# Syclus123/xDeepFM-pytorch

Measured on AMD Instinct MI355X. Metric: examples/sec (xDeepFM train step, Criteo-shape synthetic, bs=4096 per GPU), higher is better.
Workload: dtype f32

## Files before the change

xdeepfm-pytorch_amd/csrc/api.hip:

```cpp
#include <stdlib.h>
#include <string.h>
#include <algorithm>
#include <vector>
#include "xdfm_internal.h"
#include "finish_batch.h"

static thread_local char g_err[512] = "";
static int g_opts[OPT_COUNT] = {
     1,
     0,
     1,
     0,
     0,
     1,
     0,
     0,
     0,
     0,
     0,
     -1,
     -1,
     -1,
     0,
     1,
     1,
     -1,
     -1,
     -1,
     -1,
     -1,
     -1,
     1,
     -1,
     0,
     1,
     7,
     -1,
     -1,
     -1,
};
static const char* const g_opt_names[OPT_COUNT] = {"fwd_nf", "bww_nsplit", "bww_slab", "bww_mt", "dbg", "cin_math", "x3_fwd_mt", "x3_bwx_rows", "x3_waves", "bww_phase", "adam_bx", "last_fwd_kernel", "last_bwx_kernel", "last_bww_kernel", "last_sym", "x3_sym", "bww_xcd", "last_fwd_inst", "last_bwx_inst", "last_bww_inst", "last_fwd_f32", "last_bwx_f32", "last_bww_f32", "adam_rows", "last_adam_rows", "opt_bx", "finish_batch", "colaunch", "last_colaunch", "last_riders", "last_pack_riders"};

int xdfm_fail(int code, const char* fmt, ...) {
    va_list ap;
    va_start(ap, fmt);
    vsnprintf(g_err, sizeof(g_err), fmt, ap);
    va_end(ap);
    return code;
}

int xdfm_opt(int idx) { return g_opts[idx]; }

#define XDFM_MAX_DEVICES 16
void xdfm_opt_note(int idx, int value) { g_opts[idx] = value; }

__global__ __launch_bounds__(FINISH_THREADS) void finish_multi_kernel(const FinishTable tab) {
    __shared__ float smf[FINISH_THREADS];
    __shared__ double smd[4];
    int ji = 0;
#pragma unroll
    for (int k = 1; k < FINISH_MAX_JOBS; ++k) ji += (int)blockIdx.x >= tab.first[k] ? 1 : 0;
    const FinishJob& j = tab.j[ji];
    const int lb = (int)blockIdx.x - tab.first[ji];
    bool scalar_out = false;
    switch (j.kind) {
        case FJ_CIN_DBIAS:
            cin_dbias_finish_row(lb * FINISH_THREADS + (int)threadIdx.x, (const float*)j.part, j.i0, j.i1, (float*)j.out, j.i2 != 0);
            break;
        case FJ_DENSE_W:
            if (lb < j.i1) dn_finish_elem((long)lb * FINISH_THREADS + threadIdx.x, (const float*)j.part, j.i0, j.n0, j.n1, (float*)j.out, (float*)j.out2);
            else dn_dalpha_finish_block((const double*)j.part2, j.i2, (float*)j.out3, smd);
            break;
        case FJ_COLSUM:
            colsum_finish_block(lb, (const float*)j.part, j.i0, (float*)j.out, smf);
            break;
        case FJ_HEAD_FWD:
            head_fwd_finish_block((const float*)j.part, smf);
            if (threadIdx.x == 0) ((float*)j.out)[0] = smf[0];
            scalar_out = true;
            break;
        case FJ_HEAD_BWD:
            head_bwd_finish_elem(lb * FINISH_THREADS + (int)threadIdx.x, (const float*)j.part, j.i0, (float*)j.out);
            break;
        case FJ_ADAM_L2:
            adam_l2_finish_block<FINISH_THREADS>((const float*)j.part, j.i0, smf);
            if (threadIdx.x == 0) {
                ((float*)j.out)[0] = smf[0];
                if (j.cell) adam_rows_finish_one(j.cell, (float*)j.out);
            }
            scalar_out = true;
            break;
        case FJ_ADAM_ROWS:
            if (threadIdx.x == 0) adam_rows_finish_one(j.cell, (float*)j.out);
            scalar_out = true;
            break;
        default:
            scalar_out = true;
            break;
    }
    if (scalar_out && threadIdx.x == 0 && j.add_out) j.add_out[0] = j.add_a[0] + j.add_b[0];
}

struct FinishBatch {
    std::vector<FinishJob> jobs;
    hipStream_t st = nullptr;
};
static FinishBatch g_finish[XDFM_MAX_DEVICES];
static int g_finish_dev = -1;

static bool finish_job_writes(const FinishJob& j, const void* p) {
    return p && (j.out == p || j.out2 == p || j.out3 == p || (const void*)j.add_out == p || (const void*)j.cell == p);
}

static int finish_launch_pending(FinishBatch& fb) {
    const size_t n = fb.jobs.size();
    for (size_t j0 = 0; j0 < n; j0 += FINISH_MAX_JOBS) {
        FinishTable tab;
        memset(&tab, 0, sizeof(tab));
        tab.n = (int)(n - j0 < FINISH_MAX_JOBS ? n - j0 : FINISH_MAX_JOBS);
        std::stable_sort(fb.jobs.begin() + j0, fb.jobs.begin() + j0 + tab.n,
                         [](const FinishJob& a, const FinishJob& b) { return a.blocks < b.blocks; });
        int blocks = 0;
        for (int k = 0; k < tab.n; ++k) {
            tab.j[k] = fb.jobs[j0 + k];
            tab.first[k] = blocks;
            blocks += tab.j[k].blocks;
        }
        for (int k = tab.n; k <= FINISH_MAX_JOBS; ++k) tab.first[k] = blocks;
        if (blocks > 0) hipLaunchKernelGGL(finish_multi_kernel, dim3(blocks), dim3(FINISH_THREADS), 0, fb.st, tab);
    }
    fb.jobs.clear();
    return xdfm_check_launch("finish_batch");
}

int xdfm_finish_defer(const FinishJob& job, hipStream_t st, bool* taken) {
    *taken = false;
    if (g_finish_dev < 0) return XDFM_OK;
    int dev = -1;
    if (hipGetDevice(&dev) != hipSuccess || dev != g_finish_dev)
        return xdfm_fail(XDFM_ERR_INVALID, "finish batch: opened on device %d, a finish arrives on device %d", g_finish_dev, dev);
    FinishBatch& fb = g_finish[dev];
    if (fb.jobs.empty()) fb.st = st;
    else if (fb.st != st)
        return xdfm_fail(XDFM_ERR_INVALID, "finish batch: a finish arrives on stream %p, the batch collects on stream %p", (void*)st, (void*)fb.st);
    XDFM_REQUIRE(job.blocks > 0 && job.kind >= 0 && job.kind < FJ_KINDS, "finish batch: bad job (kind %d, %d workgroups)", job.kind, job.blocks);
    *taken = true;
    if (job.kind == FJ_ADAM_ROWS && job.out)
        for (size_t k = fb.jobs.size(); k-- > 0;)
            if (fb.jobs[k].kind == FJ_ADAM_L2 && fb.jobs[k].out == job.out && !fb.jobs[k].cell && !fb.jobs[k].add_out) {
                fb.jobs[k].cell = job.cell;
                return XDFM_OK;
            }
    if (job.kind == FJ_ADD)
        for (size_t k = fb.jobs.size(); k-- > 0;) {
            FinishJob& p = fb.jobs[k];
            if ((p.kind == FJ_ADAM_L2 || p.kind == FJ_ADAM_ROWS) && p.out && p.out == (const void*)job.add_b && !p.add_out &&
                !finish_job_writes(p, job.add_a)) {
                p.add_a = job.add_a; p.add_b = job.add_b; p.add_out = job.add_out;
                return XDFM_OK;
            }
        }
    const void* reads[4] = {nullptr, nullptr, nullptr, nullptr};
    if (job.kind == FJ_ADAM_ROWS) { reads[0] = job.out; reads[1] = job.cell; }
    if (job.kind == FJ_ADD) { reads[0] = job.add_a; reads[1] = job.add_b; }
    if (job.kind == FJ_CIN_DBIAS && !job.i2) reads[0] = job.out;
    reads[2] = job.out; reads[3] = job.add_out;
    bool clash = false;
    for (const FinishJob& p : fb.jobs)
        for (const void* r : reads) clash = clash || finish_job_writes(p, r);
    if (clash)
        if (int rc = finish_launch_pending(fb)) return rc;
    fb.jobs.push_back(job);
    return XDFM_OK;
}

__global__ void finish_add_kernel(const float* a, const float* b, float* out) {
    if (threadIdx.x == 0 && blockIdx.x == 0) out[0] = a[0] + b[0];
}

extern "C" {

int xdfm_abi_version(void) { return XDFM_ABI_VERSION; }

const char* xdfm_last_error(void) { return g_err; }

int xdfm_device_count(void) {
    int n = 0;
    hipError_t e = hipGetDeviceCount(&n);
    return e == hipSuccess ? n : -(int)e;
}

int xdfm_graph_node_census(void* graph, int* n_nodes, int* n_memset, int* n_unexpected) {
    if (!graph || !n_nodes || !n_memset || !n_unexpected) return xdfm_fail(XDFM_ERR_INVALID, "graph_node_census: null pointer");
    size_t n = 0;
// ... 119 lines not shown
```

xdeepfm-pytorch_amd/csrc/embed.hip:

```cpp
#include "xdfm_internal.h"
#include "cin_x3_pack.h"
#include "rider.h"

#define EMB_THREADS 256

template <int VEC>
__global__ __launch_bounds__(EMB_THREADS) void embed_gather_kernel(
    const float* __restrict__ X, long ldx, int B, const float* const* __restrict__ tables,
    const float* const* __restrict__ lin_tables, const int* __restrict__ cols, const int* __restrict__ vocab,
    int m, int D, const int* __restrict__ dense_cols, const float* __restrict__ dense_w, int nd, int EB,
    float* __restrict__ emb_fm, float* __restrict__ dnn_in, long ldd, int dense_off, float* __restrict__ lin_out,
    int* __restrict__ err_flag, int own_blocks, const X3PackJobs riders) {
    if ((int)blockIdx.x >= own_blocks) { x3_pack_rider(riders, (long)((int)blockIdx.x - own_blocks)); return; }
    extern __shared__ __attribute__((aligned(16))) float smem[];
    float* tile = smem;
    float* linv = smem + (size_t)EB * m * D;
    const float** rowp = reinterpret_cast<const float**>(smem + ((((size_t)EB * m * (D + 1)) + 1) & ~(size_t)1));
    float* densev = reinterpret_cast<float*>(rowp + (size_t)EB * m);
    float* wl = densev + (size_t)EB * nd;
    const int tid = threadIdx.x;
    const int b0 = blockIdx.x * EB;
    const int nb = (B - b0 < EB) ? B - b0 : EB;
    const int DV = D / VEC;
    const long N = (long)B * D;

    const int ndense = nb * nd;
    float dval[2] = {0.f, 0.f};
    float wval = 0.f;
    if (nd > 0) {
#pragma unroll
        for (int t = 0; t < 2; ++t) {
            const int idx = tid + t * EMB_THREADS;
            const int c = idx < ndense ? idx : 0;
            const int bl = c / nd, k = c - bl * nd;
            dval[t] = X[(long)(b0 + bl) * ldx + dense_cols[k]];
        }
        if (dense_w) wval = dense_w[tid < nd ? tid : 0];
    }
    const int npass = m <= 32 ? (nb + 7) / 8 : (nb * m + EMB_THREADS - 1) / EMB_THREADS;
    for (int p = 0; p < npass; ++p) {
        int jf, bl;
        if (m <= 32) { jf = tid & 31; bl = (tid >> 5) + 8 * p; }
        else { const int rj = tid + p * EMB_THREADS; bl = rj / m; jf = rj - bl * m; }
        const bool live = jf < m && bl < nb;
        const int jc = live ? jf : 0, bc = live ? bl : 0;
        const float* tab = tables[jc];
        const float* ltab = lin_tables ? lin_tables[jc] : tab;
        const int V = vocab[jc];
        long id = (long)X[(long)(b0 + bc) * ldx + cols[jc]];
        if (id < 0 || id >= V) {
            if (err_flag && live) atomicOr(err_flag, 1);
            id = id < 0 ? 0 : V - 1;
        }
        const float lv = ltab[lin_tables ? id : 0];
        if (live) {
            rowp[bl * m + jf] = tab + id * D;
            if (lin_tables) linv[bl * m + jf] = lv;
        }
    }
    if (nd > 0) {
#pragma unroll
        for (int t = 0; t < 2; ++t)
            if (tid + t * EMB_THREADS < ndense) densev[tid + t * EMB_THREADS] = dval[t];
        for (int idx = tid + 2 * EMB_THREADS; idx < ndense; idx += EMB_THREADS) {
            const int bl = idx / nd, k = idx - bl * nd;
            densev[idx] = X[(long)(b0 + bl) * ldx + dense_cols[k]];
        }
        if (dense_w) {
            if (tid < nd) wl[tid] = wval;
            for (int k = tid + EMB_THREADS; k < nd; k += EMB_THREADS) wl[k] = dense_w[k];
        }
    }
    __syncthreads();
    const int nchunks = nb * m * DV;
    const bool dv_pow2 = (DV & (DV - 1)) == 0;
    const int dv_sh = 31 - __builtin_clz(DV);
    constexpr int GB = 8;
    for (int base = 0; base < nchunks; base += GB * EMB_THREADS) {
        float4 v[GB];
        int at[GB];
#pragma unroll
        for (int k = 0; k < GB; ++k) {
            const int idx = base + k * EMB_THREADS + tid;
            const int cidx = idx < nchunks ? idx : nchunks - 1;
            const int rj = dv_pow2 ? (cidx >> dv_sh) : (cidx / DV);
            const int q = cidx - rj * DV;
            const float* src = rowp[rj] + q * VEC;
            at[k] = idx < nchunks ? rj * D + q * VEC : -1;
            if constexpr (VEC == 4) {
                v[k] = *reinterpret_cast<const float4*>(src);
            } else if constexpr (VEC == 2) {
                const float2 t = *reinterpret_cast<const float2*>(src);
                v[k] = make_float4(t.x, t.y, 0.f, 0.f);
            } else {
                v[k] = make_float4(*src, 0.f, 0.f, 0.f);
            }
        }
#pragma unroll
        for (int k = 0; k < GB; ++k) {
            if (at[k] < 0) continue;
            float* dst = tile + at[k];
            if constexpr (VEC == 4) *reinterpret_cast<float4*>(dst) = v[k];
            else if constexpr (VEC == 2) *reinterpret_cast<float2*>(dst) = make_float2(v[k].x, v[k].y);
            else *dst = v[k].x;
        }
    }
    __syncthreads();

    if (dnn_in) {
        const int per = m * D;
        for (int bl = 0; bl < nb; ++bl) {
            float* drow = dnn_in + (long)(b0 + bl) * ldd;
            const float* trow = tile + (size_t)bl * per;
            for (int k = tid; k < per; k += EMB_THREADS) drow[k] = trow[k];
            for (int k = tid; k < nd; k += EMB_THREADS) drow[dense_off + k] = densev[bl * nd + k];
        }
    }
    {
        const int per = nb * D;
        const bool d_pow2 = (D & (D - 1)) == 0;
        const int d_sh = 31 - __builtin_clz(D);
        for (int k = tid; k < per; k += EMB_THREADS) {
            const int bl = d_pow2 ? (k >> d_sh) : (k / D);
            const float* src = tile + (size_t)bl * m * D + (k - bl * D);
            float* dst = emb_fm + (long)b0 * D + k;
            for (int j = 0; j < m; ++j) dst[(long)j * N] = src[j * D];
        }
    }
    if (lin_out && tid < nb) {
        float acc = 0.f;
        if (lin_tables)
            for (int j = 0; j < m; ++j) acc += linv[tid * m + j];
        float dacc = 0.f;
        for (int k = 0; k < nd; ++k) dacc += densev[tid * nd + k] * wl[k];
        lin_out[b0 + tid] = acc + dacc;
    }
}

#define SC_THREADS 512
#define SC_ROWS 4096
#define SC_W 8
#define SC_SW 4
#define SC_RIDER_BLOCKS 512
#define SC_NC 4
#define SC_EMPTY 0xffffffffu

typedef float f4u __attribute__((ext_vector_type(4), aligned(4)));

__device__ __forceinline__ int sc_scale_exp(float amax) {
    const int E = (int)((__float_as_uint(amax) >> 23) & 0xff);
    return 37 - ((E == 0 ? 1 : E) - 127);
}
__device__ __forceinline__ double sc_pow2(int s) { return __longlong_as_double((long long)(1023 + s) << 52); }
__device__ __forceinline__ double sc_fix(float v, double sc) { return __builtin_rint((double)v * sc); }

__host__ __device__ inline size_t sc_lds_bytes(int npad) {
    const size_t hash = (size_t)2 * npad * 2 * sizeof(unsigned);
    const size_t slots = (size_t)(npad / SC_W) * 2 * (SC_NC * (sizeof(double) + sizeof(float)) + 2 * sizeof(int));
    return (hash > slots ? hash : slots) + (size_t)(npad + 8) * (sizeof(unsigned) + sizeof(unsigned short)) + 64 +
           (size_t)npad * 4 * sizeof(float);
}

static_assert(sizeof(X3UnpackRiders) + 512 <= 8192, "embed_scatter_grouped_kernel's argument block");
template <int VEC>
__global__ __launch_bounds__(SC_THREADS) void embed_scatter_grouped_kernel(
    const float* __restrict__ X, long ldx, int b0, int nb, long Btot, const int* __restrict__ cols,
    const int* __restrict__ vocab, int m, int D, int nslice, const float* __restrict__ d_emb_fm,
    const float* __restrict__ d_dnn_in, long ld_dnn, const float* __restrict__ d_lin, long ld_lin,
    float* __restrict__ d_flat, const long* __restrict__ tab_off, const long* __restrict__ lin_off,
    unsigned char* __restrict__ marks, int npad, int nlin, const int* __restrict__ dense_cols, int nd,
    float* __restrict__ d_dense_w, long dense_mark_base, int dbg, int own_blocks, const X3UnpackRiders riders) {
    if ((int)blockIdx.x >= own_blocks) { x3_unpack_rider(riders, (long)((int)blockIdx.x - own_blocks)); return; }
    extern __shared__ __attribute__((aligned(16))) char sc_smem[];
    const int tid = threadIdx.x;

    if ((int)blockIdx.x >= m * nslice + nlin) {
        const int k = blockIdx.x - m * nslice - nlin;
        const int col = dense_cols[k];
        float* red = reinterpret_cast<float*>(sc_smem);
        double* redd = reinterpret_cast<double*>(sc_smem + 64);
        constexpr int PER = SC_ROWS / SC_THREADS;
        float p[PER];
        float mx = 0.f;
#pragma unroll
        for (int t = 0; t < PER; ++t) {
            const int bl = tid + t * SC_THREADS;
            const long b = b0 + (bl < nb ? bl : 0);
            const float x = X[b * ldx + col], g = d_lin[b * ld_lin];
            p[t] = bl < nb ? x * g : 0.f;
            mx = fmaxf(mx, fabsf(p[t]));
        }
        for (int o = 32; o > 0; o >>= 1) mx = fmaxf(mx, __shfl_xor(mx, o));
        if ((tid & 63) == 0) red[tid >> 6] = mx;
        __syncthreads();
        mx = 0.f;
#pragma unroll
        for (int t = 0; t < SC_THREADS / 64; ++t) mx = fmaxf(mx, red[t]);
        const int s = sc_scale_exp(mx);
        const double sc = sc_pow2(s);
        double acc = 0.0;
#pragma unroll
        for (int t = 0; t < PER; ++t) acc += sc_fix(p[t], sc);
        for (int o = 32; o > 0; o >>= 1) acc += __shfl_xor(acc, o);
        if ((tid & 63) == 0) redd[tid >> 6] = acc;
        __syncthreads();
        if (tid == 0) {
            acc = 0.0;
#pragma unroll
            for (int t = 0; t < SC_THREADS / 64; ++t) acc += redd[t];
            d_dense_w[k] += (float)(acc * sc_pow2(-s));
            if (marks) marks[(dense_mark_base + k) >> 2] = 1;
        }
        return;
    }

    const bool lin = (int)blockIdx.x >= m * nslice;
    const int j = lin ? (int)blockIdx.x - m * nslice : (int)blockIdx.x / nslice;
    const int slice = lin ? 0 : (int)blockIdx.x - j * nslice;
    const int nwin = npad / SC_W;
    const int HS = 2 * npad;
    unsigned* tkey = reinterpret_cast<unsigned*>(sc_smem);
    unsigned* tcnt = tkey + HS;
    double* seqS = reinterpret_cast<double*>(sc_smem);
    float* seqM = reinterpret_cast<float*>(seqS + (size_t)2 * nwin * SC_NC);
    int* seqN = reinterpret_cast<int*>(seqM + (size_t)2 * nwin * SC_NC);
    int* seqH = seqN + 2 * nwin;
    const size_t hash_b = (size_t)HS * 2 * sizeof(unsigned), slot_b = (size_t)nwin * 2 * (SC_NC * 12 + 8);
    unsigned* gid = reinterpret_cast<unsigned*>(sc_smem + (hash_b > slot_b ? hash_b : slot_b));
    unsigned short* gb = reinterpret_cast<unsigned short*>(gid + npad + 8);
    unsigned* wsum = reinterpret_cast<unsigned*>(gb + npad + 8);
    float4* tile = reinterpret_cast<float4*>(reinterpret_cast<char*>(wsum) + 64);

    const int c0 = slice * SC_SW;
    constexpr int KPT = SC_ROWS / SC_THREADS;
    float4 pe[KPT], pd[KPT];
    {
        const bool skip = (dbg & 2) != 0;
#pragma unroll
        for (int n = 0; n < KPT; ++n) { pe[n] = make_float4(0.f, 0.f, 0.f, 0.f); pd[n] = pe[n]; }
        if (lin) {
            if (!skip) {
#pragma unroll
                for (int n = 0; n < KPT; ++n) {
                    const int i = tid + n * SC_THREADS;
                    pe[n].x = d_lin[(long)(b0 + (i < nb ? i : 0)) * ld_lin];
                }
            }
        } else {
            if (d_emb_fm && !skip) {
#pragma unroll
                for (int n = 0; n < KPT; ++n) {
                    const int i = tid + n * SC_THREADS;
                    const float* src = d_emb_fm + ((long)j * Btot + b0 + (i < nb ? i : 0)) * D;
                    if (VEC == 4) pe[n] = *reinterpret_cast<const float4*>(src + c0);
                    else pe[n] = make_float4(src[c0 < D ? c0 : D - 1], src[c0 + 1 < D ? c0 + 1 : D - 1],
                                             src[c0 + 2 < D ? c0 + 2 : D - 1], src[c0 + 3 < D ? c0 + 3 : D - 1]);
                }
            }
            if (d_dnn_in && !skip) {
#pragma unroll
                for (int n = 0; n < KPT; ++n) {
                    const int i = tid + n * SC_THREADS;
                    const float* src = d_dnn_in + (long)(b0 + (i < nb ? i : 0)) * ld_dnn + (long)j * D;
                    if (VEC == 4) { const f4u t = *reinterpret_cast<const f4u*>(src + c0); pd[n] = make_float4(t.x, t.y, t.z, t.w); }
                    else pd[n] = make_float4(src[c0 < D ? c0 : D - 1], src[c0 + 1 < D ? c0 + 1 : D - 1],
                                             src[c0 + 2 < D ? c0 + 2 : D - 1], src[c0 + 3 < D ? c0 + 3 : D - 1]);
                }
            }
        }
    }

    {
        const int V = vocab[j];
        const int col = cols[j];
        float xv[KPT];
#pragma unroll
        for (int n = 0; n < KPT; ++n) {
            const int i = tid + n * SC_THREADS;
            xv[n] = (dbg & 16) ? (float)((i * 7) % V) : X[(long)(b0 + (i < nb ? i : 0)) * ldx + col];
        }
        for (int h = tid; h < HS; h += SC_THREADS) { tkey[h] = SC_EMPTY; tcnt[h] = 0; }
        for (int i = nb + tid; i < npad + 8; i += SC_THREADS) { gid[i] = SC_EMPTY; gb[i] = 0; }
        __syncthreads();
        unsigned ids[KPT];
        int slot[KPT];
        const int hshift = 32 - (31 - __builtin_clz(HS));
        unsigned hh[KPT], step[KPT];
        bool todo[KPT];
#pragma unroll
        for (int n = 0; n < KPT; ++n) {
            const int i = tid + n * SC_THREADS;
            long id = (long)xv[n];
            id = id < 0 ? 0 : (id >= V ? V - 1 : id);
            ids[n] = (unsigned)id;
            slot[n] = 0;
            hh[n] = (ids[n] * 2654435761u) >> hshift;
            step[n] = ((ids[n] * 0x85ebca6bu) >> 15) | 1u;
            todo[n] = i < nb && !(dbg & 1);
            if (i < nb && (dbg & 1)) { gid[i] = ids[n]; gb[i] = (unsigned short)i; }
        }
        if (!(dbg & 1)) {
            for (;;) {
                unsigned prev[KPT];
#pragma unroll
                for (int n = 0; n < KPT; ++n) prev[n] = atomicCAS(&tkey[hh[n]], SC_EMPTY, ids[n]);
                bool any = false;
#pragma unroll
                for (int n = 0; n < KPT; ++n) {
                    const bool ok = prev[n] == SC_EMPTY || prev[n] == ids[n];
                    hh[n] = ok ? hh[n] : ((hh[n] + step[n]) & (HS - 1));
                    any = any || !ok;
                }
                if (!__any(any)) break;
            }
#pragma unroll
            for (int n = 0; n < KPT; ++n) {
                slot[n] = (int)hh[n];
                atomicAdd(&tcnt[hh[n]], (tid + n * SC_THREADS < nb) ? 1u : 0u);
            }
        }
        (void)todo;
        __syncthreads();
        if (!(dbg & 1)) {
            const int PER = HS >= SC_THREADS ? HS / SC_THREADS : 1;
            const int s0 = tid * PER;
            unsigned loc = 0;
            if (s0 < HS)
                for (int q = 0; q < PER; ++q) loc += tcnt[s0 + q];
            unsigned inc = loc;
            const int lane = tid & 63;
            for (int o = 1; o < 64; o <<= 1) {
                const unsigned t = __shfl_up(inc, o);
                if (lane >= o) inc += t;
            }
            if (lane == 63) wsum[tid >> 6] = inc;
            __syncthreads();
            unsigned basew = 0;
            for (int q = 0; q < (tid >> 6); ++q) basew += wsum[q];
            unsigned run = basew + inc - loc;
            if (s0 < HS)
                for (int q = 0; q < PER; ++q) { const unsigned c = tcnt[s0 + q]; tcnt[s0 + q] = run; run += c; }
            __syncthreads();
            unsigned pos[KPT];
#pragma unroll
            for (int n = 0; n < KPT; ++n) pos[n] = atomicAdd(&tcnt[slot[n]], (tid + n * SC_THREADS < nb) ? 1u : 0u);
#pragma unroll
            for (int n = 0; n < KPT; ++n) {
                const int i = tid + n * SC_THREADS;
                if (i < nb) { gid[pos[n]] = ids[n]; gb[pos[n]] = (unsigned short)i; }
            }
        }
        __syncthreads();
    }

    const int w = tid;
    const int base = w * SC_W;
    const bool live = base < nb;
    const int count = live ? (nb - base < SC_W ? nb - base : SC_W) : 0;
    unsigned id[SC_W];
    int bl[SC_W];
    {
        const int bs = live ? base : 0;
        const uint4 i0 = *reinterpret_cast<const uint4*>(gid + bs), i1 = *reinterpret_cast<const uint4*>(gid + bs + 4);
        const uint4 bb = *reinterpret_cast<const uint4*>(gb + bs);
        const unsigned iv[8] = {i0.x, i0.y, i0.z, i0.w, i1.x, i1.y, i1.z, i1.w};
        const unsigned bv[8] = {bb.x & 0xffffu, bb.x >> 16, bb.y & 0xffffu, bb.y >> 16, bb.z & 0xffffu, bb.z >> 16, bb.w & 0xffffu, bb.w >> 16};
#pragma unroll
        for (int q = 0; q < SC_W; ++q) {
            id[q] = live ? iv[q] : SC_EMPTY;
            bl[q] = q < count ? (int)bv[q] : 0;
        }
    }
    const bool contL = live && base > 0 && gid[base - 1] == id[0];
    const bool contR = count == SC_W && base + SC_W < nb && gid[base + SC_W] == id[SC_W - 1];
    const bool single = id[0] == id[SC_W - 1];
    const bool owner = contR && !(contL && single);
#pragma unroll
    for (int n = 0; n < KPT; ++n) {
        const int i = tid + n * SC_THREADS;
        if (i < npad) tile[i] = make_float4(pe[n].x + pd[n].x, pe[n].y + pd[n].y, pe[n].z + pd[n].z, pe[n].w + pd[n].w);
    }
    const bool any_open = __syncthreads_or(contR) != 0;

    const long row_base = lin ? (lin_off ? lin_off[j] : -1) : (tab_off ? tab_off[j] : -1);
    const bool vrow = !lin && VEC == 4 && row_base >= 0 && ((row_base & 3) == 0);
    float4 old[SC_W];
#pragma unroll
    for (int q = 0; q < SC_W; ++q) old[q] = make_float4(0.f, 0.f, 0.f, 0.f);
    if (row_base >= 0 && !(dbg & 4)) {
        if (vrow) {
#pragma unroll
            for (int q = 0; q < SC_W; ++q)
                old[q] = *reinterpret_cast<const float4*>(d_flat + row_base + (long)(q < count ? id[q] : 0u) * D + c0);
        } else if (lin) {
#pragma unroll
            for (int q = 0; q < SC_W; ++q) old[q].x = d_flat[row_base + (long)(q < count ? id[q] : 0u)];
        }
    }
    float v[SC_W][SC_NC];
#pragma unroll
    for (int q = 0; q < SC_W; ++q) {
        const float4 t = tile[bl[q]];
        const float tv[4] = {t.x, t.y, t.z, t.w};
#pragma unroll
        for (int c = 0; c < 4; ++c) v[q][c] = (q < count && (lin ? c == 0 : c0 + c < D)) ? tv[c] : 0.f;
    }

    float pm[SC_W][SC_NC];
#pragma unroll
    for (int q = 0; q < SC_W; ++q)
#pragma unroll
        for (int c = 0; c < SC_NC; ++c) {
            const float a = fabsf(v[q][c]);
            pm[q][c] = (q > 0 && id[q] == id[q - 1]) ? fmaxf(pm[q - 1][c], a) : a;
        }
#pragma unroll
    for (int q = SC_W - 2; q >= 0; --q)
#pragma unroll
        for (int c = 0; c < SC_NC; ++c)
            if (q + 1 < count && id[q] == id[q + 1]) pm[q][c] = pm[q + 1][c];
    float res[SC_W][SC_NC];
    bool fin[SC_W];
    {
        double acc[SC_NC];
#pragma unroll
        for (int q = 0; q < SC_W; ++q) {
            const bool first = q == 0 || id[q] != id[q - 1];
            const bool last = q == count - 1 || (q < count && id[q] != id[q + 1 < SC_W ? q + 1 : q]);
            const bool pieceL = contL && id[q] == id[0];
            const bool pieceR = contR && id[q] == id[SC_W - 1];
            fin[q] = q < count && last && !pieceL && !pieceR && !(dbg & 4);
#pragma unroll
            for (int c = 0; c < SC_NC; ++c) {
                const int s = sc_scale_exp(pm[q][c]);
                const double f = sc_fix(v[q][c], sc_pow2(s));
                acc[c] = first ? f : acc[c] + f;
                res[q][c] = (float)(acc[c] * sc_pow2(-s));
            }
            if (any_open && q < count && last && (pieceL || pieceR)) {
#pragma unroll
                for (int c = 0; c < SC_NC; ++c) seqM[(size_t)(2 * w + (pieceL ? 0 : 1)) * SC_NC + c] = pm[q][c];
            }
        }
    }
    if (row_base >= 0) {
#pragma unroll
        for (int q = 0; q < SC_W; ++q) {
            if (fin[q]) {
                if (vrow) {
                    const long e = row_base + (long)id[q] * D + c0;
                    *reinterpret_cast<float4*>(d_flat + e) = make_float4(old[q].x + res[q][0], old[q].y + res[q][1],
                                                                         old[q].z + res[q][2], old[q].w + res[q][3]);
                    if (marks) marks[e >> 2] = 1;
                } else if (lin) {
                    const long e = row_base + (long)id[q];
                    d_flat[e] = old[q].x + res[q][0];
                    if (marks) marks[e >> 2] = 1;
                } else {
#pragma unroll
                    for (int c = 0; c < 4; ++c)
                        if (c0 + c < D) {
                            const long e = row_base + (long)id[q] * D + c0 + c;
                            d_flat[e] += res[q][c];
                            if (marks) marks[e >> 2] = 1;
                        }
                }
            }
        }
    }
    if (!any_open || (dbg & 8)) return;
    const bool both = contL && contR && single;
    const bool act = w < nwin;
    const int e0 = act ? 2 * w : 0, e1 = act ? 2 * w + 1 : 0;
    if (act) {
        const bool hasL = live && contL, hasR = live && contR && !both;
        if (!hasL) {
#pragma unroll
            for (int c = 0; c < SC_NC; ++c) seqM[(size_t)e0 * SC_NC + c] = 0.f;
        }
        if (!hasR) {
#pragma unroll
            for (int c = 0; c < SC_NC; ++c) seqM[(size_t)e1 * SC_NC + c] = 0.f;
        }
        seqN[e0] = both ? e1 : -1;
        seqN[e1] = (live && contR) ? e1 + 1 : -1;
        seqH[e0] = (live && contL) ? e0 - 1 : e0;
        seqH[e1] = both ? e0 : e1;
    }
    __syncthreads();
    float4* seqM4 = reinterpret_cast<float4*>(seqM);
    for (;;) {
        const int n0 = act ? seqN[e0] : -1, n1 = act ? seqN[e1] : -1, h0 = seqH[e0], h1 = seqH[e1];
        const int nn0 = n0 >= 0 ? seqN[n0] : -1, nn1 = n1 >= 0 ? seqN[n1] : -1;
        const int hh0 = seqH[h0], hh1 = seqH[h1];
        const float4 z4 = make_float4(0.f, 0.f, 0.f, 0.f);
        const float4 m0 = n0 >= 0 ? seqM4[n0] : z4, m1 = n1 >= 0 ? seqM4[n1] : z4;
        const float4 o0 = seqM4[e0], o1 = seqM4[e1];
        const bool more = act && (n0 >= 0 || n1 >= 0 || hh0 != h0 || hh1 != h1);
        if (!__syncthreads_or(more)) break;
        if (act) {
            seqM4[e0] = make_float4(fmaxf(o0.x, m0.x), fmaxf(o0.y, m0.y), fmaxf(o0.z, m0.z), fmaxf(o0.w, m0.w));
            seqM4[e1] = make_float4(fmaxf(o1.x, m1.x), fmaxf(o1.y, m1.y), fmaxf(o1.z, m1.z), fmaxf(o1.w, m1.w));
            seqN[e0] = nn0; seqN[e1] = nn1; seqH[e0] = hh0; seqH[e1] = hh1;
        }
        __syncthreads();
    }
    int sL[SC_NC], sR[SC_NC];
    {
        const int h0 = seqH[e0], h1 = seqH[e1];
        double aL[SC_NC], aR[SC_NC];
#pragma unroll
        for (int c = 0; c < SC_NC; ++c) {
            sL[c] = sc_scale_exp(seqM[(size_t)h0 * SC_NC + c]);
            sR[c] = sc_scale_exp(seqM[(size_t)h1 * SC_NC + c]);
            aL[c] = 0.0; aR[c] = 0.0;
        }
#pragma unroll
        for (int q = 0; q < SC_W; ++q) {
            const bool inL = contL && q < count && id[q] == id[0];
            const bool inR = contR && !both && id[q] == id[SC_W - 1];
#pragma unroll
            for (int c = 0; c < SC_NC; ++c) {
                if (inL) aL[c] += sc_fix(v[q][c], sc_pow2(sL[c]));
                if (inR) aR[c] += sc_fix(v[q][c], sc_pow2(sR[c]));
            }
        }
        if (act) {
#pragma unroll
            for (int c = 0; c < SC_NC; ++c) {
                seqS[(size_t)e0 * SC_NC + c] = aL[c];
                seqS[(size_t)e1 * SC_NC + c] = aR[c];
            }
            seqN[e0] = both ? e1 : -1;
            seqN[e1] = (live && contR) ? e1 + 1 : -1;
        }
    }
    __syncthreads();
    double2* seqS2 = reinterpret_cast<double2*>(seqS);
    for (;;) {
        const int n0 = act ? seqN[e0] : -1, n1 = act ? seqN[e1] : -1;
        const int nn0 = n0 >= 0 ? seqN[n0] : -1, nn1 = n1 >= 0 ? seqN[n1] : -1;
        const double2 z2 = make_double2(0.0, 0.0);
        const double2 a0l = n0 >= 0 ? seqS2[2 * n0] : z2, a0h = n0 >= 0 ? seqS2[2 * n0 + 1] : z2;
        const double2 a1l = n1 >= 0 ? seqS2[2 * n1] : z2, a1h = n1 >= 0 ? seqS2[2 * n1 + 1] : z2;
        const double2 o0l = seqS2[2 * e0], o0h = seqS2[2 * e0 + 1], o1l = seqS2[2 * e1], o1h = seqS2[2 * e1 + 1];
        if (!__syncthreads_or(n0 >= 0 || n1 >= 0)) break;
        if (act) {
            seqS2[2 * e0] = make_double2(o0l.x + a0l.x, o0l.y + a0l.y); seqS2[2 * e0 + 1] = make_double2(o0h.x + a0h.x, o0h.y + a0h.y);
            seqS2[2 * e1] = make_double2(o1l.x + a1l.x, o1l.y + a1l.y); seqS2[2 * e1 + 1] = make_double2(o1h.x + a1h.x, o1h.y + a1h.y);
            seqN[e0] = nn0; seqN[e1] = nn1;
        }
        __syncthreads();
    }
    if (owner && row_base >= 0) {
        const unsigned rid = id[SC_W - 1];
        float r[SC_NC];
#pragma unroll
        for (int c = 0; c < SC_NC; ++c) r[c] = (float)(seqS[(size_t)e1 * SC_NC + c] * sc_pow2(-sR[c]));
        if (lin) {
            const long e = row_base + (long)rid;
            d_flat[e] += r[0];
            if (marks) marks[e >> 2] = 1;
        } else {
#pragma unroll
            for (int c = 0; c < 4; ++c)
                if (c0 + c < D) {
                    const long e = row_base + (long)rid * D + c0 + c;
                    d_flat[e] += r[c];
                    if (marks) marks[e >> 2] = 1;
                }
        }
    }
}

extern "C" {

int xdfm_embed_gather_fwd(const float* X, long ldx, int B, const float* const* tables,
                          const float* const* lin_tables, const int* cols, const int* vocab, int m, int D,
                          const int* dense_cols, const float* dense_w, int nd, float* emb_fm, float* dnn_in,
                          float* lin_out, int* err_flag, void* stream) {
    return xdfm_embed_gather_fwd_ld(X, ldx, B, tables, lin_tables, cols, vocab, m, D, dense_cols, dense_w, nd, emb_fm, dnn_in,
                                    (long)m * D + nd, m * D, lin_out, err_flag, stream);
}

int xdfm_embed_gather_fwd_ld(const float* X, long ldx, int B, const float* const* tables,
                             const float* const* lin_tables, const int* cols, const int* vocab, int m, int D,
                             const int* dense_cols, const float* dense_w, int nd, float* emb_fm, float* dnn_in,
                             long ld_dnn, int dense_off, float* lin_out, int* err_flag, void* stream) {
    XDFM_REQUIRE(X && tables && cols && vocab && emb_fm, "embed_gather_fwd: null pointer");
    XDFM_REQUIRE(B > 0 && m > 0 && D > 0 && nd >= 0 && ldx >= m + nd, "embed_gather_fwd: bad shape B=%d m=%d D=%d nd=%d ldx=%ld",
                 B, m, D, nd, ldx);
    XDFM_REQUIRE(nd == 0 || dense_cols, "embed_gather_fwd: dense_cols missing");
    XDFM_REQUIRE(!(lin_out && nd > 0) || dense_w, "embed_gather_fwd: dense_w missing");
    XDFM_REQUIRE(!dnn_in || (dense_off >= (long)m * D && ld_dnn >= (long)dense_off + nd),
                 "embed_gather_fwd: bad dnn_in layout ld_dnn=%ld dense_off=%d (m*D=%ld, nd=%d)", ld_dnn, dense_off, (long)m * D, nd);
    int EB = (int)(8192 / ((long)m * D));
    if (EB > 16) EB = 16;
    if (xdfm_opt(OPT_DBG) & 1024) { EB = (int)(16384 / ((long)m * D)); if (EB > 32) EB = 32; }
    if ((xdfm_opt(OPT_DBG) & 256) && EB > 4) EB = 4;
    if ((xdfm_opt(OPT_DBG) & 512) && EB > 8) EB = 8;
    if (EB < 1) EB = 1;
    const size_t lds = ((size_t)EB * m * D + (size_t)EB * m) * sizeof(float) + (size_t)EB * m * sizeof(void*) + 8 +
                       ((size_t)EB * nd + (size_t)nd) * sizeof(float);
    XDFM_REQUIRE(lds <= 160 * 1024, "embed_gather_fwd: m*D=%ld too large for one LDS tile", (long)m * D);
    XDFM_REQUIRE(EB <= EMB_THREADS, "embed_gather_fwd: internal");
    dim3 grid(ceil_div(B, EB));
    hipStream_t st = (hipStream_t)stream;
    static_assert(EMB_THREADS == 256, "the pack bodies' grid is counted in 256-thread workgroups");
    const int own_blocks = (int)grid.x;
    X3PackJobs riders = {};
    grid.x += (unsigned)x3_pack_take_pack(st, &riders);
#define LAUNCH(V)                                                                                              \
    hipLaunchKernelGGL((embed_gather_kernel<V>), grid, dim3(EMB_THREADS), lds, st, X, ldx, B, tables, lin_tables, \
                       cols, vocab, m, D, dense_cols, dense_w, nd, EB, emb_fm, dnn_in, ld_dnn, dense_off, lin_out, err_flag, \
                       own_blocks, riders)
    if (D % 4 == 0) LAUNCH(4);
    else if (D % 2 == 0) LAUNCH(2);
    else LAUNCH(1);
#undef LAUNCH
    return xdfm_check_launch("embed_gather_fwd");
}

int xdfm_embed_scatter_bwd(const float* X, long ldx, int B, const int* cols, const int* vocab, int m, int D,
                           const int* dense_cols, int nd, const float* d_emb_fm, const float* d_dnn_in,
                           const float* d_lin, float* d_flat, const long* tab_off, const long* lin_off,
                           float* d_dense_w, void* stream) {
    return xdfm_embed_scatter_bwd_marked(X, ldx, B, cols, vocab, m, D, dense_cols, nd, d_emb_fm, d_dnn_in, 0, d_lin, 0,
                                         d_flat, tab_off, lin_off, d_dense_w, nullptr, stream);
}

int xdfm_embed_scatter_bwd_marked(const float* X, long ldx, int B, const int* cols, const int* vocab, int m, int D,
                                  const int* dense_cols, int nd, const float* d_emb_fm, const float* d_dnn_in,
                                  long ld_dnn, const float* d_lin, long ld_lin, float* d_flat, const long* tab_off,
                                  const long* lin_off, float* d_dense_w, unsigned char* marks, void* stream) {
    XDFM_REQUIRE(X && cols && vocab, "embed_scatter_bwd: null pointer");
    if (ld_dnn <= 0) ld_dnn = (long)m * D + nd;
    if (ld_lin <= 0) ld_lin = 1;
    XDFM_REQUIRE(ld_dnn >= (long)m * D, "embed_scatter_bwd: ld_dnn %ld smaller than m*D", ld_dnn);
    XDFM_REQUIRE(!marks || (d_flat && (((size_t)d_flat) & 15) == 0), "embed_scatter_bwd: marks need a 16-byte aligned d_flat");
    XDFM_REQUIRE(!marks || !d_dense_w || d_dense_w >= d_flat, "embed_scatter_bwd: with marks d_dense_w must lie inside d_flat");
    XDFM_REQUIRE(d_flat || (!tab_off && !lin_off), "embed_scatter_bwd: offsets without a gradient buffer");
    XDFM_REQUIRE(B > 0 && m > 0 && D > 0 && nd >= 0, "embed_scatter_bwd: bad shape");
    hipStream_t st = (hipStream_t)stream;
    const bool tabs = tab_off != nullptr;
    const bool lins = d_lin && lin_off;
    const bool dense = nd > 0 && d_lin && d_dense_w;
    if (dense) XDFM_REQUIRE(dense_cols, "embed_scatter_bwd: dense_cols missing");
    if (!tabs && !lins && !dense) return XDFM_OK;
    XDFM_REQUIRE(!tabs || d_emb_fm || d_dnn_in, "embed_scatter_bwd: table offsets without row gradients");
    const bool vec4 = D % 4 == 0 && ((((size_t)d_flat) | ((size_t)d_emb_fm)) & 15) == 0 && !(xdfm_opt(OPT_DBG) & 2048);
    const int nslice = tabs ? ceil_div(D, SC_SW) : 0;
    const int nlin = lins ? m : 0;
    for (long b0 = 0; b0 < B; b0 += SC_ROWS) {
        const int nb = (int)(B - b0 < SC_ROWS ? B - b0 : SC_ROWS);
        int npad = 8;
        while (npad < nb) npad <<= 1;
        const size_t lds = sc_lds_bytes(npad);
        dim3 grid(m * nslice + nlin + (dense ? nd : 0));
        const int own_blocks = (int)grid.x;
        X3UnpackRiders riders = {};
        if (b0 == 0) grid.x += (unsigned)x3_riders_take(st, SC_THREADS, SC_RIDER_BLOCKS, &riders);
        const long mark_base = marks && dense ? (long)(d_dense_w - d_flat) : 0L;
        const int dbg = (xdfm_opt(OPT_DBG) >> 12) & 31;
        if (vec4)
            hipLaunchKernelGGL((embed_scatter_grouped_kernel<4>), grid, dim3(SC_THREADS), lds, st, X, ldx, (int)b0, nb, (long)B,
                               cols, vocab, m, D, nslice, d_emb_fm, d_dnn_in, ld_dnn, d_lin, ld_lin, d_flat, tab_off, lin_off,
                               marks, npad, nlin, dense_cols, dense ? nd : 0, d_dense_w, mark_base, dbg, own_blocks, riders);
        else
            hipLaunchKernelGGL((embed_scatter_grouped_kernel<1>), grid, dim3(SC_THREADS), lds, st, X, ldx, (int)b0, nb, (long)B,
                               cols, vocab, m, D, nslice, d_emb_fm, d_dnn_in, ld_dnn, d_lin, ld_lin, d_flat, tab_off, lin_off,
                               marks, npad, nlin, dense_cols, dense ? nd : 0, d_dense_w, mark_base, dbg, own_blocks, riders);
        const int rc = xdfm_check_launch("embed_scatter_bwd");
        if (rc) return rc;
    }
    return XDFM_OK;
}

}
```

xdeepfm-pytorch_amd/csrc/xdfm_internal.h:

```cpp
#pragma once
#include <hip/hip_runtime.h>
#include <stdarg.h>
#include <stdio.h>
#include "../../include/xdfm.h"

typedef float f32x16 __attribute__((ext_vector_type(16)));
typedef float f32x4 __attribute__((ext_vector_type(4)));

#define XDFM_WAVE 64

int xdfm_fail(int code, const char* fmt, ...);
int xdfm_opt(int idx);
void xdfm_opt_note(int idx, int value);
enum {
    OPT_FWD_NF = 0,
    OPT_BWW_NSPLIT,
    OPT_BWW_SLAB,
    OPT_BWW_MT,
    OPT_DBG,
    OPT_CIN_MATH,
    OPT_X3_FWD_MT,
    OPT_X3_BWX_ROWS,
    OPT_X3_WAVES,
    OPT_BWW_PHASE,
    OPT_ADAM_BX,
    OPT_LAST_FWD,
    OPT_LAST_BWX,
    OPT_LAST_BWW,
    OPT_LAST_SYM,
    OPT_X3_SYM,
    OPT_BWW_XCD,
    OPT_LAST_FWD_INST,
    OPT_LAST_BWX_INST,
    OPT_LAST_BWW_INST,
    OPT_LAST_FWD_F32,
    OPT_LAST_BWX_F32,
    OPT_LAST_BWW_F32,
    OPT_ADAM_ROWS,
    OPT_LAST_ADAM_ROWS,
    OPT_OPT_BX,
    OPT_FINISH_BATCH,
    OPT_COLAUNCH,
    OPT_LAST_COLAUNCH,
    OPT_LAST_RIDERS,
    OPT_LAST_PACK_RIDERS,
    OPT_COUNT
};
static inline int x3_inst_code(int T, int NW, int NT, bool SYM) { return T * 1000 + NW * 100 + NT * 10 + (SYM ? 1 : 0); }
static inline int f32_fwd_code(int MT, int NF, int MPT) { return MT * 1000 + NF * 100 + MPT; }
static inline int f32_bwx_code(int HS4, int JB) { return HS4 * 10 + JB; }
static inline int f32_bww_code(int MT, int KV, bool slab, int nsplit) { return nsplit * 1000 + MT * 100 + KV * 10 + (slab ? 1 : 0); }

#ifdef __HIPCC__
__device__ __forceinline__ float xdfm_sigmoid(float v) { return 1.f / (1.f + expf(-v)); }
__device__ __forceinline__ float xdfm_sigmoid_slope(float y) { return fmaf(-y, y, y); }
__device__ __forceinline__ float xdfm_act_bwd(int act, float a, float g) {
    if (act == XDFM_ACT_RELU) return a > 0.f ? g : 0.f;
    if (act == XDFM_ACT_SIGMOID) return g * xdfm_sigmoid_slope(a);
    return g;
}
__device__ __forceinline__ double xdfm_block_sum_f64(double v, double* sm) {
#pragma unroll
    for (int off = 32; off >= 1; off >>= 1) v += __shfl_xor(v, off);
    if ((threadIdx.x & 63) == 0) sm[threadIdx.x >> 6] = v;
    __syncthreads();
    double s = sm[0];
    for (int w = 1; w < (int)(blockDim.x >> 6); ++w) s += sm[w];
    return s;
}
__device__ __forceinline__ unsigned drop_mix(unsigned x) {
    x ^= x >> 16; x *= 0x7feb352dU; x ^= x >> 15; x *= 0x846ca68bU; x ^= x >> 16;
    return x;
}
#endif
static inline unsigned xdfm_drop_thresh(float p_drop) {
    const double t = (double)p_drop * 4294967296.0;
    return t >= 4294967295.0 ? 4294967295u : (unsigned)t;
}
static inline float xdfm_drop_keep_scale(float p_drop) { return 1.0f / (1.0f - p_drop); }
static inline bool xdfm_act_known(int act) { return act == XDFM_ACT_LINEAR || act == XDFM_ACT_RELU || act == XDFM_ACT_SIGMOID; }

#define XDFM_REQUIRE(cond, ...) \
    do { if (!(cond)) return xdfm_fail(XDFM_ERR_INVALID, __VA_ARGS__); } while (0)

static inline int xdfm_check_launch(const char* what) {
    hipError_t e = hipGetLastError();
    if (e != hipSuccess) return xdfm_fail(XDFM_ERR_LAUNCH, "%s: %s", what, hipGetErrorString(e));
    return XDFM_OK;
}

int xdfm_opt_step_dense(int kind, const char* what, const xdfm_opt_tensor* tensors, int T, double lr, const double* lr_dev, double eps,
                        double alpha, double mu, int nesterov, float* l2_ws, float* l2_value, void* stream);

static inline int ceil_div(long a, long b) { return (int)((a + b - 1) / b); }
static inline long round_up(long a, long b) { return (a + b - 1) / b * b; }

static inline int fwd_mt(int H) {
    int t = ceil_div(H, 32);
    if (t >= 8) return 8;
    if (t > 2) return 4;
    return t;
}
#define FWD_PD 3
#define BWX_PD 3
#define BWX_TAIL(hs4) (2 * (hs4) + BWX_PD)
static inline int fwd_mp(int m) { return (m + 1) / 2; }
static inline long fwd_tpad(int Hp, int m) { return round_up((long)Hp * fwd_mp(m), 4); }
static inline int bwx_hs4(int H) {
    int g = ceil_div(H, 8);
    int p = 1;
    while (p < g) p <<= 1;
    return p;
}

__device__ __forceinline__ int frag_row(int r, int s) { return (r & 3) + 8 * (r >> 2) + 4 * s; }

static inline int x3_terms() { const int m = xdfm_opt(OPT_CIN_MATH); return m == 1 ? 3 : (m == 2 ? 1 : 0); }
#define X3_HDR 128
#define X3_RING 4
#define X3_STAGE_KB 16
#define X3_BWX_RING 4
constexpr __host__ __device__ inline int x3_fwd_sps(int MT, int nt, int m) {
    const int stepkb = (nt == 3 ? 2 : 1) * MT;
    int sps = X3_STAGE_KB / stepkb;
    if (sps < 1) sps = 1;
    const int lim = (m / 2 - 1) / (X3_RING - 1);
    while (sps > 1 && sps > lim) sps >>= 1;
    return sps;
}
constexpr __host__ __device__ inline int x3_sym_pairs(int m) { return (m / 2) * (m / 2 + 1); }
constexpr __host__ __device__ inline int x3_sym_steps(int m) { return (x3_sym_pairs(m) + 7) / 8; }
constexpr __host__ __device__ inline int x3_sym_i(int m, int q) {
    int i = 0;
    while (i < m / 2 && q >= m - 2 * i) { q -= m - 2 * i; ++i; }
    return i;
}
constexpr __host__ __device__ inline int x3_sym_j(int m, int q) {
    int i = 0;
    while (i < m / 2 && q >= m - 2 * i) { q -= m - 2 * i; ++i; }
    return i + q;
}
constexpr __host__ __device__ inline int x3_fwd_sps_sym(int MT, int nt) {
    const int sps = X3_STAGE_KB / ((nt == 3 ? 2 : 1) * MT);
    return sps < 1 ? 1 : sps;
}
static inline bool x3_sym_m(int m) { return m == 22 || m == 26; }
struct X3Geom {
    int MT, MB;
    int MP;
    int FB, RH, TS, NS;
    int SPS, NSA;
};
struct X3FwdEpi {
    int keep_rows;
    float* res; long ldres; int res_off, dir0, logD;
    unsigned* mask; long mask_ld;
};
static inline X3FwdEpi x3_fwd_epi_plain(int H) { return X3FwdEpi{H, nullptr, 0, 0, 0, 0, nullptr, 0}; }
X3Geom x3_fwd_geom(int H, int Hp, int m);
X3Geom x3_fwd_geom_sym(int H, int m);
bool x3_fwd_usable(int H, int Hp, int m);
size_t x3_fwd_pack_elems(int H, int Hp, int m);
int x3_fwd_pack(const float* W, int H, int Hp, int m, float* pack, hipStream_t st);
int x3_level_fwd(const float* xp, const float* x0, const float* pack, const float* bias, int H, int Hp, int m, long N,
                 int act, float* out, const X3FwdEpi& epi, hipStream_t st);
int x3_level_fwd_sym(const float* x0, const float* pack, const float* bias, int H, int m, long N, const X3Geom& g, int nt,
                     int act, float* out, const X3FwdEpi& epi, hipStream_t st);
int x3_level_fwd_ma(const float* xp, const float* x0, const float* pack, const float* bias, int H, int Hp, int m, long N,
                    const X3Geom& g, int nt, int act, float* out, const X3FwdEpi& epi, hipStream_t st);
int x3_level_fwd_mb(const float* xp, const float* x0, const float* pack, const float* bias, int H, int Hp, int m, long N,
                    const X3Geom& g, int nt, int act, float* out, const X3FwdEpi& epi, hipStream_t st);
struct X3BwxGeom {
    int HBT, HBS, IB;
    long NT;
};
struct X3DoutSrc {
    const float* dOut;
    const unsigned* mask; long mask_ld;
    const float* dHid; int hid_rows;
    const float* dDir; int dir_mode; long lddir; int dir_off, dir0, dir_rows, logD;
    int h0;
};
static inline X3DoutSrc x3_dout_plain(const float* dOut) { return X3DoutSrc{dOut, nullptr, 0, nullptr, 0, nullptr, 0, 0, 0, 0, 0, 0, 0}; }
X3BwxGeom x3_bwx_geom(int H, int Hp, int m);
bool x3_bwx_usable(int H, int Hp, int m);
size_t x3_bwx_pack_elems(int H, int Hp, int m);
int x3_bwx_pack(const float* W, int H, int Hp, int m, float* pack, hipStream_t st);
int x3_level_bwd_x(const X3DoutSrc& S, const float* xp, const float* x0, const float* pack, int H, int Hp, int m, long N,
                   float* dxp, float* dx0, int flags, hipStream_t st);

int x3_level_bwd_x_sym(const X3DoutSrc& S, const float* x0, const float* pack, int H, int m, long N, int HBT, int nt,
                       float* dxp, float* dx0, int flags, hipStream_t st);

#define BWW_NC 32
static inline int bww_mt(int H) {
    const int o = xdfm_opt(OPT_BWW_MT);
    if (o == 1 || o == 2 || o == 4) return o;
    return H > 64 ? 4 : (H > 32 ? 2 : 1);
// ... 61 lines not shown
```

Baseline: 2.176 million.

## Replace embedding-grad segment merge with wave-level segmented scans in scatter kernel

Adds a templated K2 mode to the grouped embedding-gradient scatter kernel. The default setting (2) replaces the existing window-merge path with wave-level segmented max/sum scans plus a cross-wave LDS carry, computing fixed-point scaled run sums per row. Bit 1 adds wave-aggregated hash insertion for hot IDs to reduce LDS atomic contention, but it is off by default. The change is meant to cut serial merging and synchronisation in the backward scatter, at the cost of more shuffles and extra __syncthreads.

```diff
diff --git a/xdeepfm-pytorch_amd/csrc/api.hip b/xdeepfm-pytorch_amd/csrc/api.hip
--- a/xdeepfm-pytorch_amd/csrc/api.hip
+++ b/xdeepfm-pytorch_amd/csrc/api.hip
@@ -38,8 +38,9 @@
      -1,
      -1,
      -1,
+     2,
 };
-static const char* const g_opt_names[OPT_COUNT] = {"fwd_nf", "bww_nsplit", "bww_slab", "bww_mt", "dbg", "cin_math", "x3_fwd_mt", "x3_bwx_rows", "x3_waves", "bww_phase", "adam_bx", "last_fwd_kernel", "last_bwx_kernel", "last_bww_kernel", "last_sym", "x3_sym", "bww_xcd", "last_fwd_inst", "last_bwx_inst", "last_bww_inst", "last_fwd_f32", "last_bwx_f32", "last_bww_f32", "adam_rows", "last_adam_rows", "opt_bx", "finish_batch", "colaunch", "last_colaunch", "last_riders", "last_pack_riders"};
+static const char* const g_opt_names[OPT_COUNT] = {"fwd_nf", "bww_nsplit", "bww_slab", "bww_mt", "dbg", "cin_math", "x3_fwd_mt", "x3_bwx_rows", "x3_waves", "bww_phase", "adam_bx", "last_fwd_kernel", "last_bwx_kernel", "last_bww_kernel", "last_sym", "x3_sym", "bww_xcd", "last_fwd_inst", "last_bwx_inst", "last_bww_inst", "last_fwd_f32", "last_bwx_f32", "last_bww_f32", "adam_rows", "last_adam_rows", "opt_bx", "finish_batch", "colaunch", "last_colaunch", "last_riders", "last_pack_riders", "k2"};
 
 int xdfm_fail(int code, const char* fmt, ...) {
     va_list ap;
diff --git a/xdeepfm-pytorch_amd/csrc/embed.hip b/xdeepfm-pytorch_amd/csrc/embed.hip
--- a/xdeepfm-pytorch_amd/csrc/embed.hip
+++ b/xdeepfm-pytorch_amd/csrc/embed.hip
@@ -161,8 +161,44 @@
            (size_t)npad * 4 * sizeof(float);
 }
 
+#define SC_HOT_R 3
+#define SC_HOT_MIN 4
+__device__ __forceinline__ void sc_hot_masks(unsigned key, unsigned long long (&gm)[SC_HOT_R]) {
+    unsigned long long rem = ~0ull;
+#pragma unroll
+    for (int r = 0; r < SC_HOT_R; ++r) {
+        gm[r] = 0;
+        if (rem) {
+            const unsigned lead = (unsigned)__builtin_amdgcn_readlane((int)key, __ffsll(rem) - 1);
+            const unsigned long long mk = __ballot(key == lead);
+            rem &= ~mk;
+            if (__popcll(mk) >= SC_HOT_MIN) gm[r] = mk;
+        }
+    }
+}
+__device__ __forceinline__ float sc_op(float a, float b) { return fmaxf(a, b); }
+__device__ __forceinline__ double sc_op(double a, double b) { return a + b; }
+template <typename T>
+__device__ __forceinline__ void sc_seg_scan_left(T (&v)[SC_NC], int lane, int rl) {
+#pragma unroll
+    for (int o = 1; o < 64; o <<= 1) {
+        const bool take = rl >= o && lane >= o;
+#pragma unroll
+        for (int c = 0; c < SC_NC; ++c) { const T t = __shfl_up(v[c], o); v[c] = take ? sc_op(v[c], t) : v[c]; }
+    }
+}
+template <typename T>
+__device__ __forceinline__ void sc_seg_scan_right(T (&v)[SC_NC], int lane, int rr) {
+#pragma unroll
+    for (int o = 1; o < 64; o <<= 1) {
+        const bool take = rr >= o && lane + o < 64;
+#pragma unroll
+        for (int c = 0; c < SC_NC; ++c) { const T t = __shfl_down(v[c], o); v[c] = take ? sc_op(v[c], t) : v[c]; }
+    }
+}
+
 static_assert(sizeof(X3UnpackRiders) + 512 <= 8192, "embed_scatter_grouped_kernel's argument block");
-template <int VEC>
+template <int VEC, int K2>
 __global__ __launch_bounds__(SC_THREADS) void embed_scatter_grouped_kernel(
     const float* __restrict__ X, long ldx, int b0, int nb, long Btot, const int* __restrict__ cols,
     const int* __restrict__ vocab, int m, int D, int nslice, const float* __restrict__ d_emb_fm,
@@ -299,11 +335,32 @@
             todo[n] = i < nb && !(dbg & 1);
             if (i < nb && (dbg & 1)) { gid[i] = ids[n]; gb[i] = (unsigned short)i; }
         }
+        constexpr bool AGG = (K2 & 1) != 0;
+        constexpr int NG = AGG ? SC_HOT_R : 1;
+        const int lane = tid & 63;
+        unsigned long long gm[KPT][NG], vb[KPT];
+        bool own[KPT];
+#pragma unroll
+        for (int n = 0; n < KPT; ++n) {
+            own[n] = true;
+            if constexpr (AGG) {
+                sc_hot_masks(ids[n], gm[n]);
+                vb[n] = __ballot(tid + n * SC_THREADS < nb);
+#pragma unroll
+                for (int r = 0; r < NG; ++r)
+                    if (gm[n][r]) own[n] = own[n] && (!((gm[n][r] >> lane) & 1) || lane == __ffsll(gm[n][r]) - 1);
+            }
+        }
         if (!(dbg & 1)) {
             for (;;) {
                 unsigned prev[KPT];
 #pragma unroll
-                for (int n = 0; n < KPT; ++n) prev[n] = atomicCAS(&tkey[hh[n]], SC_EMPTY, ids[n]);
+                for (int n = 0; n < KPT; ++n) {
+                    if constexpr (AGG) {
+                        prev[n] = ids[n];
+                        if (own[n]) prev[n] = atomicCAS(&tkey[hh[n]], SC_EMPTY, ids[n]);
+                    } else prev[n] = atomicCAS(&tkey[hh[n]], SC_EMPTY, ids[n]);
+                }
                 bool any = false;
 #pragma unroll
                 for (int n = 0; n < KPT; ++n) {
@@ -315,11 +372,26 @@
             }
 #pragma unroll
             for (int n = 0; n < KPT; ++n) {
-                slot[n] = (int)hh[n];
-                atomicAdd(&tcnt[hh[n]], (tid + n * SC_THREADS < nb) ? 1u : 0u);
-            }
-        }
-        (void)todo;
+                unsigned add = (tid + n * SC_THREADS < nb) ? 1u : 0u;
+                if constexpr (AGG) {
+#pragma unroll
+                    for (int r = 0; r < NG; ++r)
+                        if (gm[n][r]) {
+                            const int ld = __ffsll(gm[n][r]) - 1;
+                            const unsigned lh = (unsigned)__builtin_amdgcn_readlane((int)hh[n], ld);
+                            const bool in = (gm[n][r] >> lane) & 1;
+                            hh[n] = in ? lh : hh[n];
+                            add = in ? (unsigned)__popcll(gm[n][r] & vb[n]) : add;
+                        }
+                    slot[n] = (int)hh[n];
+                    if (own[n]) atomicAdd(&tcnt[hh[n]], add);
+                } else {
+                    slot[n] = (int)hh[n];
+                    atomicAdd(&tcnt[hh[n]], add);
+                }
+            }
+        }
+        (void)todo; (void)gm; (void)vb; (void)own; (void)lane;
         __syncthreads();
         if (!(dbg & 1)) {
             const int PER = HS >= SC_THREADS ? HS / SC_THREADS : 1;
@@ -343,7 +415,27 @@
             __syncthreads();
             unsigned pos[KPT];
 #pragma unroll
-            for (int n = 0; n < KPT; ++n) pos[n] = atomicAdd(&tcnt[slot[n]], (tid + n * SC_THREADS < nb) ? 1u : 0u);
+            for (int n = 0; n < KPT; ++n) {
+                unsigned add = (tid + n * SC_THREADS < nb) ? 1u : 0u;
+                if constexpr (AGG) {
+#pragma unroll
+                    for (int r = 0; r < NG; ++r)
+                        if (gm[n][r]) add = ((gm[n][r] >> lane) & 1) ? (unsigned)__popcll(gm[n][r] & vb[n]) : add;
+                    pos[n] = 0;
+                    if (own[n]) pos[n] = atomicAdd(&tcnt[slot[n]], add);
+                } else pos[n] = atomicAdd(&tcnt[slot[n]], add);
+            }
+            if constexpr (AGG) {
+#pragma unroll
+                for (int n = 0; n < KPT; ++n)
+#pragma unroll
+                    for (int r = 0; r < NG; ++r)
+                        if (gm[n][r]) {
+                            const unsigned lp = (unsigned)__builtin_amdgcn_readlane((int)pos[n], __ffsll(gm[n][r]) - 1);
+                            const unsigned rank = (unsigned)__popcll(gm[n][r] & vb[n] & ((1ull << lane) - 1ull));
+                            pos[n] = ((gm[n][r] >> lane) & 1) ? lp + rank : pos[n];
+                        }
+            }
 #pragma unroll
             for (int n = 0; n < KPT; ++n) {
                 const int i = tid + n * SC_THREADS;
@@ -472,6 +564,117 @@
     const bool both = contL && contR && single;
     const bool act = w < nwin;
     const int e0 = act ? 2 * w : 0, e1 = act ? 2 * w + 1 : 0;
+    if constexpr ((K2 & 2) != 0) {
+        const int lane = tid & 63, wv = tid >> 6;
+        const int nwl = (nwin + 63) >> 6;
+        float* xF = reinterpret_cast<float*>(sc_smem);
+        float* xS = xF + nwl * SC_NC;
+        unsigned long long* xO = reinterpret_cast<unsigned long long*>(xS + nwl * SC_NC);
+        double* xD = reinterpret_cast<double*>(xO + nwl);
+        const bool hasL = live && contL, hasR = live && contR && !both;
+        float mL[SC_NC], mR[SC_NC], F[SC_NC], S[SC_NC];
+#pragma unroll
+        for (int c = 0; c < SC_NC; ++c) {
+            mL[c] = hasL ? seqM[(size_t)e0 * SC_NC + c] : 0.f;
+            mR[c] = hasR ? seqM[(size_t)e1 * SC_NC + c] : 0.f;
+            F[c] = both ? mL[c] : mR[c];
+            S[c] = mL[c];
+        }
+        const unsigned long long ones = __ballot(both);
+        const unsigned long long zl = ~ones << (63 - lane), zr = ~ones >> lane;
+        const int rl = zl ? __clzll(zl) : lane + 1;
+        const int rr = zr ? __ffsll(zr) - 1 : 64 - lane;
+        sc_seg_scan_left(F, lane, rl);
+        sc_seg_scan_right(S, lane, rr);
+        if (wv < nwl) {
+            if (lane == 63) {
+#pragma unroll
+                for (int c = 0; c < SC_NC; ++c) xF[wv * SC_NC + c] = F[c];
+            }
+            if (lane == 0) {
+#pragma unroll
+                for (int c = 0; c < SC_NC; ++c) xS[wv * SC_NC + c] = S[c];
+                xO[wv] = ones;
+            }
+        }
+        __syncthreads();
+        float tF[SC_NC], tS[SC_NC];
+#pragma unroll
+        for (int c = 0; c < SC_NC; ++c) { tF[c] = 0.f; tS[c] = 0.f; }
+        if (wv < nwl) {
+            for (int k = wv - 1; k >= 0; --k) {
+#pragma unroll
+                for (int c = 0; c < SC_NC; ++c) tF[c] = fmaxf(tF[c], xF[k * SC_NC + c]);
+                if (xO[k] != ~0ull) break;
+            }
+            for (int k = wv + 1; k < nwl; ++k) {
+#pragma unroll
+                for (int c = 0; c < SC_NC; ++c) tS[c] = fmaxf(tS[c], xS[k * SC_NC + c]);
+                if (xO[k] != ~0ull) break;
+            }
+        }
+        int sL[SC_NC], sR[SC_NC];
+#pragma unroll
+        for (int c = 0; c < SC_NC; ++c) {
+            const float f = rl == lane + 1 ? fmaxf(F[c], tF[c]) : F[c], s = rr == 64 - lane ? fmaxf(S[c], tS[c]) : S[c];
+            const float fp = __shfl_up(f, 1), sn = __shfl_down(s, 1);
+            const float fprev = lane == 0 ? tF[c] : fp, snext = lane == 63 ? tS[c] : sn;
+            sL[c] = sc_scale_exp(both ? fmaxf(f, s) : fmaxf(fprev, mL[c]));
+            sR[c] = sc_scale_exp(fmaxf(mR[c], snext));
+        }
+        double aL[SC_NC], aR[SC_NC];
+#pragma unroll
+        for (int c = 0; c < SC_NC; ++c) { aL[c] = 0.0; aR[c] = 0.0; }
+#pragma unroll
+        for (int q = 0; q < SC_W; ++q) {
+            const bool inL = contL && q < count && id[q] == id[0];
+            const bool inR = contR && !both && id[q] == id[SC_W - 1];
+#pragma unroll
+            for (int c = 0; c < SC_NC; ++c) {
+                if (inL) aL[c] += sc_fix(v[q][c], sc_pow2(sL[c]));
+                if (inR) aR[c] += sc_fix(v[q][c], sc_pow2(sR[c]));
+            }
+        }
+        sc_seg_scan_right(aL, lane, rr);
+        if (wv < nwl && lane == 0) {
+#pragma unroll
+            for (int c = 0; c < SC_NC; ++c) xD[wv * SC_NC + c] = aL[c];
+        }
+        __syncthreads();
+        double tD[SC_NC];
+#pragma unroll
+        for (int c = 0; c < SC_NC; ++c) tD[c] = 0.0;
+        if (wv < nwl)
+            for (int k = wv + 1; k < nwl; ++k) {
+#pragma unroll
+                for (int c = 0; c < SC_NC; ++c) tD[c] += xD[k * SC_NC + c];
+                if (xO[k] != ~0ull) break;
+            }
+        float r[SC_NC];
+#pragma unroll
+        for (int c = 0; c < SC_NC; ++c) {
+            const double s = rr == 64 - lane ? aL[c] + tD[c] : aL[c];
+            const double sn = __shfl_down(s, 1);
+            r[c] = (float)((aR[c] + (lane == 63 ? tD[c] : sn)) * sc_pow2(-sR[c]));
+        }
+        if (owner && row_base >= 0) {
+            const unsigned rid = id[SC_W - 1];
+            if (lin) {
+                const long e = row_base + (long)rid;
+                d_flat[e] += r[0];
+                if (marks) marks[e >> 2] = 1;
+            } else {
+#pragma unroll
+                for (int c = 0; c < 4; ++c)
+                    if (c0 + c < D) {
+                        const long e = row_base + (long)rid * D + c0 + c;
+                        d_flat[e] += r[c];
+                        if (marks) marks[e >> 2] = 1;
+                    }
+            }
+        }
+        return;
+    }
     if (act) {
         const bool hasL = live && contL, hasR = live && contR && !both;
         if (!hasL) {
@@ -662,14 +865,21 @@
         if (b0 == 0) grid.x += (unsigned)x3_riders_take(st, SC_THREADS, SC_RIDER_BLOCKS, &riders);
         const long mark_base = marks && dense ? (long)(d_dense_w - d_flat) : 0L;
         const int dbg = (xdfm_opt(OPT_DBG) >> 12) & 31;
-        if (vec4)
-            hipLaunchKernelGGL((embed_scatter_grouped_kernel<4>), grid, dim3(SC_THREADS), lds, st, X, ldx, (int)b0, nb, (long)B,
-                               cols, vocab, m, D, nslice, d_emb_fm, d_dnn_in, ld_dnn, d_lin, ld_lin, d_flat, tab_off, lin_off,
-                               marks, npad, nlin, dense_cols, dense ? nd : 0, d_dense_w, mark_base, dbg, own_blocks, riders);
-        else
-            hipLaunchKernelGGL((embed_scatter_grouped_kernel<1>), grid, dim3(SC_THREADS), lds, st, X, ldx, (int)b0, nb, (long)B,
-                               cols, vocab, m, D, nslice, d_emb_fm, d_dnn_in, ld_dnn, d_lin, ld_lin, d_flat, tab_off, lin_off,
-                               marks, npad, nlin, dense_cols, dense ? nd : 0, d_dense_w, mark_base, dbg, own_blocks, riders);
+#define LAUNCH(V, K)                                                                                                      \
+        hipLaunchKernelGGL((embed_scatter_grouped_kernel<V, K>), grid, dim3(SC_THREADS), lds, st, X, ldx, (int)b0, nb, (long)B, \
+                           cols, vocab, m, D, nslice, d_emb_fm, d_dnn_in, ld_dnn, d_lin, ld_lin, d_flat, tab_off, lin_off,     \
+                           marks, npad, nlin, dense_cols, dense ? nd : 0, d_dense_w, mark_base, dbg, own_blocks, riders)
+        switch ((vec4 ? 4 : 0) | (xdfm_opt(OPT_K2) & 3)) {
+            case 4: LAUNCH(4, 0); break;
+            case 5: LAUNCH(4, 1); break;
+            case 6: LAUNCH(4, 2); break;
+            case 7: LAUNCH(4, 3); break;
+            case 0: LAUNCH(1, 0); break;
+            case 1: LAUNCH(1, 1); break;
+            case 2: LAUNCH(1, 2); break;
+            default: LAUNCH(1, 3); break;
+        }
+#undef LAUNCH
         const int rc = xdfm_check_launch("embed_scatter_bwd");
         if (rc) return rc;
     }
diff --git a/xdeepfm-pytorch_amd/csrc/xdfm_internal.h b/xdeepfm-pytorch_amd/csrc/xdfm_internal.h
--- a/xdeepfm-pytorch_amd/csrc/xdfm_internal.h
+++ b/xdeepfm-pytorch_amd/csrc/xdfm_internal.h
@@ -44,6 +44,7 @@
     OPT_LAST_COLAUNCH,
     OPT_LAST_RIDERS,
     OPT_LAST_PACK_RIDERS,
+    OPT_K2,
     OPT_COUNT
 };
 static inline int x3_inst_code(int T, int NW, int NT, bool SYM) { return T * 1000 + NW * 100 + NT * 10 + (SYM ? 1 : 0); }
```

Result: no change. 2.194 million (median of 6 runs) (+0.8%).
